# bacpop/Pansim

Hardware: AMD Instinct MI355X
Metric: generations/sec (higher is better)
Workload: dtype u8

## Files before the change

pansim_amd/csrc/acc_kernels.h:

```cpp
#pragma once

#include "ps_common.h"

struct acc_dims { uint32_t N, G, W, GW; };

__global__ void acc_init_kernel(uint64_t *accG, uint64_t *accI, const uint8_t *init_vec, acc_dims d)
{
    const uint64_t t = (uint64_t)blockIdx.x * blockDim.x + threadIdx.x;
    const uint64_t nG = (uint64_t)d.G * d.W, nI = (uint64_t)d.N * d.GW;
    if (t < nG) {
        const uint32_t g = (uint32_t)(t / d.W), w = (uint32_t)(t % d.W);
        const uint32_t nb = min(64u, d.N - w * 64u);
        const uint64_t m = (nb == 64u) ? ~0ull : ((1ull << nb) - 1ull);
        accG[t] = init_vec[g] ? m : 0ull;
    } else if (t < nG + nI) {
        const uint64_t u = t - nG;
        const uint32_t gw = (uint32_t)(u % d.GW);
        uint64_t word = 0;
        for (uint32_t b = 0; b < 64; b++) {
            const uint32_t g = gw * 64u + b;
            if (g < d.G && init_vec[g]) word |= 1ull << b;
        }
        accI[u] = word;
    }
// ... 66 lines not shown
    const uint32_t i = (uint32_t)(t / d.GW), gw = (uint32_t)(t % d.GW);
    const uint32_t p = DO_GATHER ? a.idx[i] : i;
    if (DO_GATHER && a.idx_out && gw == 0) a.idx_out[i] = p;
    uint64_t word = a.srcI[(uint64_t)p * d.GW + gw];
    if (DO_MUT && WT) {
        const uint4 *thr = (const uint4 *)(a.gene_thr + (size_t)gw * 64u);
        uint32_t lt[2] = { 0u, 0u };
#pragma unroll
        for (uint32_t j = 0; j < 16u; j++) {
            const ps_u4 r = ps_philox(gw * 16u + j, i, a.gen, PS_STREAM_ACC_MUT, a.k0, a.k1);
            const uint4 t = thr[j];
            const uint32_t b = 4u * j;
            lt[b >> 5] |= ((r.x < t.x ? 1u : 0u) | (r.y < t.y ? 2u : 0u) | (r.z < t.z ? 4u : 0u) | (r.w < t.w ? 8u : 0u)) << (b & 31u);
        }
        word ^= ((uint64_t)lt[1] << 32) | lt[0];
    } else if (DO_MUT) {
        const uint32_t t0 = a.plan.n_comp > 0 ? a.plan.flip_thr[0] : 0u, t1 = a.plan.n_comp > 1 ? a.plan.flip_thr[1] : 0u;
        const uint64_t m0 = a.plan.n_comp > 0 ? ps_word_range_mask(gw, a.plan.comp_begin[0], a.plan.comp_end[0]) : 0ull;
        const uint64_t m1 = a.plan.n_comp > 1 ? ps_word_range_mask(gw, a.plan.comp_begin[1], a.plan.comp_end[1]) : 0ull;
        uint32_t lt0[2] = { 0u, 0u }, lt1[2] = { 0u, 0u };
#pragma unroll
        for (uint32_t j = 0; j < 16u; j++) {
            const ps_u4 r = ps_philox(gw * 16u + j, i, a.gen, PS_STREAM_ACC_MUT, a.k0, a.k1);
            const uint32_t w[4] = { r.x, r.y, r.z, r.w };
#pragma unroll
            for (uint32_t k = 0; k < 4u; k++) {
                const uint32_t b = 4u * j + k;
                lt0[b >> 5] |= (w[k] < t0 ? 1u : 0u) << (b & 31u);
                lt1[b >> 5] |= (w[k] < t1 ? 1u : 0u) << (b & 31u);
            }
        }
        const uint64_t f0 = ((uint64_t)lt0[1] << 32) | lt0[0], f1 = ((uint64_t)lt1[1] << 32) | lt1[0];
        word ^= (f1 & m1) | (f0 & m0 & ~m1);
    }
    a.dstI[t] = word;
    if (a.snapI) a.snapI[t] = word;
}

struct acc_hgt_args {
    const uint64_t *srcI;
    uint64_t *dstI;
    acc_dims d;
    uint32_t n_comp;
    uint32_t gb[PS_MAX_COMP], ge[PS_MAX_COMP];
    const uint32_t *ptab[PS_MAX_COMP];
    uint32_t kmin[PS_MAX_COMP], plen[PS_MAX_COMP];
    uint32_t *work_ctr;
    uint32_t gen, k0, k1;
    uint32_t *bins, *counts;
    uint32_t bin_cap;
    uint32_t parts, rows_per_part;
    uint32_t part_magic;
    uint32_t *scratch;
    unsigned long long *ovf_img;
    uint32_t *overflow_flag;
    uint16_t *list_scratch;
    uint32_t list_stride;
    uint32_t dn_lo, dn_cnt;
    uint32_t bin_prio;
    const uint16_t *wq[PS_MAX_COMP];
    const uint64_t *wnz[PS_MAX_COMP];
    uint32_t pref_off;
};

__device__ __forceinline__ uint32_t ps_hgt_count(const acc_hgt_args &a, uint32_t c, uint32_t dn)
{
    if (!a.ptab[c]) return 0u;
    const ps_u4 r = ps_philox(dn, 0u, a.gen, PS_STREAM_HGT_COUNT | (c << 8), a.k0, a.k1);
    uint32_t lo = 0, hi = a.plen[c];
    while (lo < hi) {
        const uint32_t mid = (lo + hi) >> 1;
        if (a.ptab[c][mid] <= r.x) lo = mid + 1u; else hi = mid;
    }
    if (lo >= a.plen[c]) lo = a.plen[c] - 1u;
    return a.kmin[c] + lo;
}

__global__ void __launch_bounds__(256) acc_snapshot_kernel(const uint64_t *copy_src, uint64_t *copy_dst, uint64_t words)
{
    for (uint64_t w = (uint64_t)blockIdx.x * blockDim.x + threadIdx.x; w < words; w += (uint64_t)gridDim.x * blockDim.x)
        copy_dst[w] = copy_src[w];
}

__device__ __forceinline__ uint32_t ps_wave_gene_list(const uint64_t *row, uint32_t GW, uint32_t gb, uint32_t ge,
                                                      uint16_t *list, uint32_t lane)
{
    uint32_t base = 0;
    for (uint32_t gw0 = gb >> 6; gw0 * 64u < ge; gw0 += 64u) {
        const uint32_t gw = gw0 + lane;
        uint64_t word = 0;
        if (gw * 64u < ge && gw < GW) {
            word = row[gw];
            const uint32_t lo = gw * 64u;
            if (lo < gb) word &= ~0ull << (gb - lo);
            if (lo + 64u > ge) word &= (ge - lo >= 64u) ? ~0ull : ((1ull << (ge - lo)) - 1ull);
        }
        const uint32_t pc = __popcll(word);
        uint32_t incl = pc;
        for (int off = 1; off < 64; off <<= 1) {
            const uint32_t t = __shfl_up(incl, off, 64);
            if ((int)lane >= off) incl += t;
        }
        uint32_t pos = base + incl - pc;
        while (word) {
            const uint32_t b = (uint32_t)__builtin_ctzll(word);
            word &= word - 1ull;
            list[pos++] = (uint16_t)(gw * 64u + b);
        }
        base += __shfl(incl, 63, 64);
    }
    return base;
}

__device__ __forceinline__ uint32_t ps_wave_gene_list_w(const uint64_t *row, uint32_t GW, uint32_t G, const uint64_t *wnz, const uint16_t *wq,
                                                        uint16_t *list, uint32_t *pref, uint32_t lane, uint32_t *total)
{
    uint32_t base = 0, wbase = 0;
    for (uint32_t gw0 = 0; gw0 * 64u < G; gw0 += 64u) {
        const uint32_t gw = gw0 + lane;
        uint64_t word = 0;
        if (gw < GW) word = row[gw] & wnz[gw];
        const uint32_t pc = __popcll(word);
        uint32_t ws = 0;
        for (uint64_t t = word; t; t &= t - 1ull) ws += wq[gw * 64u + (uint32_t)__builtin_ctzll(t)];
        uint32_t incl = pc, wincl = ws;
        for (int off = 1; off < 64; off <<= 1) {
            const uint32_t t = __shfl_up(incl, off, 64), u = __shfl_up(wincl, off, 64);
            if ((int)lane >= off) { incl += t; wincl += u; }
        }
        uint32_t pos = base + incl - pc, run = wbase + wincl - ws;
        while (word) {
            const uint32_t g = gw * 64u + (uint32_t)__builtin_ctzll(word);
            word &= word - 1ull;
            run += wq[g];
            list[pos] = (uint16_t)g;
            pref[pos++] = run;
        }
        base += __shfl(incl, 63, 64);
        wbase += __shfl(wincl, 63, 64);
    }
    *total = wbase;
    return base;
}
__device__ __forceinline__ uint32_t ps_weighted_pick(const uint32_t *pref, uint32_t n, uint32_t total, uint32_t word)
{
    const uint32_t x = ps_mulhi(word, total);
    uint32_t lo = 0, hi = n - 1u;
    while (lo < hi) {
        const uint32_t mid = (lo + hi) >> 1;
        if (pref[mid] > x) hi = mid; else lo = mid + 1u;
    }
    return lo;
}

template <bool WT = false>
__global__ void __launch_bounds__(64) acc_hgt_donor_wave_kernel(acc_hgt_args a)
{
    extern __shared__ __attribute__((aligned(16))) uint16_t lds_list[];
    uint16_t *glist = a.list_scratch ? a.list_scratch + (uint64_t)blockIdx.x * a.list_stride : lds_list;
    uint32_t *pref = (uint32_t *)(glist + a.pref_off);
    uint32_t wtotal = 0;
    const acc_dims d = a.d;
    const uint32_t lane = threadIdx.x;
    const uint32_t items = a.n_comp * a.dn_cnt;
    for (;;) {
        uint32_t item = 0;
        if (lane == 0) item = atomicAdd(a.work_ctr, 1u);
        item = __builtin_amdgcn_readfirstlane(item);
        if (item >= items) break;
        const uint32_t c = item / a.dn_cnt, dn = a.dn_lo + item % a.dn_cnt;
        const uint32_t k = ps_hgt_count(a, c, dn);
        if (k == 0u) continue;
        __threadfence_block();
        const uint32_t n = WT ? ps_wave_gene_list_w(a.srcI + (uint64_t)dn * d.GW, d.GW, d.G, a.wnz[c], a.wq[c], glist, pref, lane, &wtotal)
                              : ps_wave_gene_list(a.srcI + (uint64_t)dn * d.GW, d.GW, a.gb[c], a.ge[c], glist, lane);
        __threadfence_block();
        if (n == 0u) continue;
        const uint32_t stream = PS_STREAM_HGT | (c << 8);
        for (uint32_t jp = lane; 2u * jp < k; jp += 64u) {
            const ps_u4 r = ps_philox(jp, dn, a.gen, stream, a.k0, a.k1);
#pragma unroll
            for (uint32_t h = 0; h < 2u; h++) {
                if (2u * jp + h >= k) break;
                uint32_t rc = ps_mulhi(h ? r.z : r.x, d.N - 1u);
                rc += (rc >= dn) ? 1u : 0u;
                const uint32_t gene = glist[WT ? ps_weighted_pick(pref, n, wtotal, h ? r.w : r.y) : ps_mulhi(h ? r.w : r.y, n)];
                atomicOr((unsigned long long *)&a.dstI[(uint64_t)rc * d.GW + (gene >> 6)], 1ull << (gene & 63u));
            }
        }
    }
}

#ifndef PS_HGT_BIN_BLOCKS
#define PS_HGT_BIN_BLOCKS 2u
#endif
template <bool WT = false>
__global__ void __launch_bounds__(256) acc_hgt_donor_bin_kernel(acc_hgt_args a)
{
    extern __shared__ __attribute__((aligned(16))) uint32_t sc_lds[];
    uint32_t *fill = sc_lds;
    uint16_t *glist = a.list_scratch ? a.list_scratch + (uint64_t)blockIdx.x * a.list_stride
                                     : (uint16_t *)(sc_lds + ((a.parts + 3u) & ~3u));
    __shared__ uint32_t sh_n;
    __shared__ uint32_t sh_total;
    const uint32_t *pref = (const uint32_t *)(glist + a.pref_off);
    const acc_dims d = a.d;
    const uint32_t tid = threadIdx.x, lane = tid & 63u;
    const uint32_t items = a.n_comp * a.dn_cnt;
    const uint32_t cap = a.bin_cap;
    if (a.bin_prio >= 3u) __builtin_amdgcn_s_setprio(3);
    else if (a.bin_prio == 2u) __builtin_amdgcn_s_setprio(2);
    else if (a.bin_prio == 1u) __builtin_amdgcn_s_setprio(1);
    uint32_t *mybins = a.bins + (uint64_t)blockIdx.x * a.parts * cap;
    for (uint32_t q = tid; q < a.parts; q += blockDim.x) fill[q] = 0u;
    for (uint32_t item = blockIdx.x; item < items; item += gridDim.x) {
        __syncthreads();
        const uint32_t c = item / a.dn_cnt, dn = a.dn_lo + item % a.dn_cnt;
        const uint32_t k = ps_hgt_count(a, c, dn);
        if (k == 0u) continue;
        if (tid < 64u) {
            uint32_t tot = 0;
            const uint32_t m = WT ? ps_wave_gene_list_w(a.srcI + (uint64_t)dn * d.GW, d.GW, d.G, a.wnz[c], a.wq[c], glist, (uint32_t *)(glist + a.pref_off), lane, &tot)
                                  : ps_wave_gene_list(a.srcI + (uint64_t)dn * d.GW, d.GW, a.gb[c], a.ge[c], glist, lane);
            if (tid == 0) { sh_n = m; if (WT) sh_total = tot; }
            __threadfence_block();
        }
        __syncthreads();
        const uint32_t n = sh_n;
        if (n == 0u) continue;
        const uint32_t wtotal = WT ? sh_total : 0u;
        const uint32_t stream = PS_STREAM_HGT | (c << 8);
        auto place = [&](uint32_t rc, uint32_t gene, uint32_t part, uint32_t pos) {
            if (pos < cap) mybins[(uint64_t)part * cap + pos] = ((rc - part * a.rows_per_part) << 16) | gene;
            else atomicOr(&a.ovf_img[(uint64_t)rc * d.GW + (gene >> 6)], 1ull << (gene & 63u));
        };
        constexpr uint32_t NBK = PS_HGT_BIN_BLOCKS;
        for (uint32_t jp = tid; 2u * jp < k; jp += NBK * blockDim.x) {
            uint32_t wr[2u * NBK], wg[2u * NBK];
            bool ok[2u * NBK];
#pragma unroll
            for (uint32_t b = 0; b < NBK; b++) {
                const uint32_t jb = jp + b * blockDim.x;
                const ps_u4 r = ps_philox(jb, dn, a.gen, stream, a.k0, a.k1);
                wr[2u * b] = r.x; wg[2u * b] = r.y; wr[2u * b + 1u] = r.z; wg[2u * b + 1u] = r.w;
                ok[2u * b] = 2u * jb < k;
                ok[2u * b + 1u] = 2u * jb + 1u < k;
            }
            uint32_t rc[2u * NBK], gene[2u * NBK], part[2u * NBK], pos[2u * NBK];
#pragma unroll
            for (uint32_t e = 0; e < 2u * NBK; e++) {
                rc[e] = ps_mulhi(wr[e], d.N - 1u);
                rc[e] += (rc[e] >= dn) ? 1u : 0u;
                gene[e] = glist[WT ? ps_weighted_pick(pref, n, wtotal, wg[e]) : ps_mulhi(wg[e], n)];
                part[e] = ps_mulhi(rc[e], a.part_magic);
            }
#pragma unroll
            for (uint32_t e = 0; e < 2u * NBK; e++) pos[e] = ok[e] ? atomicAdd(&fill[part[e]], 1u) : 0u;
#pragma unroll
            for (uint32_t e = 0; e < 2u * NBK; e++)
                if (ok[e]) place(rc[e], gene[e], part[e], pos[e]);
        }
    }
    __syncthreads();
    for (uint32_t q = tid; q < a.parts; q += blockDim.x) {
        a.counts[(uint64_t)blockIdx.x * a.parts + q] = min(fill[q], cap);
    }
}

__global__ void __launch_bounds__(1024) acc_hgt_apply_kernel(acc_hgt_args a, uint32_t donor_blocks, uint32_t n_slices)
{
    extern __shared__ uint32_t lrow[];
    const acc_dims d = a.d;
// ... 913 lines not shown
```

pansim_amd/csrc/core_kernels.h:

```cpp
#pragma once

#include "ps_common.h"

#include <type_traits>

#define PS_SWEEP_MAX_GENS 2
struct core_sweep_args {
    uint8_t *state;
    uint8_t *out;
    const uint32_t *idx;
    const uint32_t *idx_next[PS_SWEEP_MAX_GENS - 1];
    const uint32_t *idxT;
    uint32_t N, pitch, cpr, rows;
    uint32_t site_offset;
    uint32_t gen, k0, k1;
    ps_core_plan plan;
    uint32_t *overflow_flag;
    unsigned long long *stamps;
    uint32_t *work_ctr;
    uint32_t launch_parity;
    uint32_t nt;
    uint32_t qcap;
    uint32_t qcap_limit;
    uint32_t *wide_flags;
// ... 200 lines not shown
                                                     uint32_t k, uint32_t nE, uint32_t vm)
{
    const uint32_t c1 = __builtin_amdgcn_bitop3_b32(p1, p2, p3, 0x01) & vm;
    uint32_t lt;
    switch (nE) {
    case 1: lt = __builtin_amdgcn_bitop3_b32(p0, p5, p4, 0x01); break;
    case 2: lt = __builtin_amdgcn_bitop3_b32(p0, p5, p4, 0x03); break;
    case 3: lt = __builtin_amdgcn_bitop3_b32(p0, p5, p4, 0x07); break;
    case 4: lt = __builtin_amdgcn_bitop3_b32(p0, p5, p4, 0x0F); break;
    case 5: lt = __builtin_amdgcn_bitop3_b32(p0, p5, p4, 0x1F); break;
    case 6: lt = __builtin_amdgcn_bitop3_b32(p0, p5, p4, 0x3F); break;
    case 7: lt = __builtin_amdgcn_bitop3_b32(p0, p5, p4, 0x7F); break;
    default: lt = 0xFFFFFFFFu; break;
    }
    ps_class_words o;
    o.dec = k ? c1 & __builtin_amdgcn_bitop3_b32(p0, p5, p4, 0x07) : 0u;
    o.res = c1 & lt & ~o.dec;
    return o;
}

struct ps_apply_words { uint32_t y0, y1, ya, yb, yc; };
PS_HD uint32_t ps_bfi(uint32_t m, uint32_t a, uint32_t b)
{
#if defined(__HIP_DEVICE_COMPILE__) && __has_builtin(__builtin_amdgcn_bitop3_b32)
    return __builtin_amdgcn_bitop3_b32(m, a, b, 0xCA);
#else
    return (a & m) | (b & ~m);
#endif
}
__device__ __forceinline__ ps_apply_words ps_apply_prepare(uint32_t dec, uint32_t p4, uint32_t p5)
{
    const uint32_t r1 = p5 >> 1, r2 = p4 >> 2, l1 = p5 << 1, l2 = dec << 2;
    ps_apply_words o;
    o.y0 = ps_bfi(0x01010101u, p4, ps_bfi(0x02020202u, l1, l2));
    o.y1 = ps_bfi(0x02020202u, p4, ps_bfi(0x04040404u, l1, l2));
    o.ya = ps_bfi(0x09090909u, r2, ps_bfi(0x12121212u, r1, dec));
    o.yb = ps_bfi(0x12121212u, r2, ps_bfi(0x24242424u, r1, dec));
    o.yc = ps_bfi(0x24242424u, r2, ps_bfi(0x48484848u, r1, dec));
    return o;
}
template <uint32_t SLOT>
__device__ __forceinline__ uint32_t ps_apply_dword(const ps_apply_words &y, uint32_t d)
{
    constexpr uint32_t sh = SLOT == 0u ? 0u : SLOT == 1u ? 1u : SLOT == 2u ? 0u : SLOT == 3u ? 1u : SLOT == 4u ? 2u : SLOT == 5u ? 3u : SLOT == 6u ? 4u : 5u;
    const uint32_t src = SLOT == 0u ? y.y0 : SLOT == 1u ? y.y1 : (SLOT == 2u || SLOT == 5u) ? y.ya : (SLOT == 3u || SLOT == 6u) ? y.yb : y.yc;
    const uint32_t f = (src >> sh) & 0x07070707u;
    const uint32_t allele = __builtin_amdgcn_perm(0x00080402u, 0u, f);
    const uint32_t mask = __builtin_amdgcn_perm(0x00FFFFFFu, 0u, f);
    return ps_bfi(mask, allele, d);
}
template <uint32_t H>
__device__ __forceinline__ void ps_apply_row(const ps_apply_words &y, uint4 &d)
{
    d.x = ps_apply_dword<4u * H + 0u>(y, d.x);
    d.y = ps_apply_dword<4u * H + 1u>(y, d.y);
    d.z = ps_apply_dword<4u * H + 2u>(y, d.z);
    d.w = ps_apply_dword<4u * H + 3u>(y, d.w);
}

__device__ __forceinline__ uint32_t ps_push_scan(uint32_t w0, uint32_t w1, uint16_t *q, uint32_t lane, uint32_t qcap)
{
    const uint32_t c0 = (uint32_t)__popc(w0), c = c0 + (uint32_t)__popc(w1);
    const uint32_t incl = ps_wave_scan_incl(c);
    const uint32_t qn = __builtin_amdgcn_readlane(incl, 63);
    if (qn <= qcap) {
        uint16_t *qp = q + (incl - c) - 1, *qp1 = qp + c0;
        const uint32_t tag = lane << 6;
        for (uint32_t m = w0; m; m &= m - 1u) *++qp = (uint16_t)(tag | (uint32_t)__builtin_ctz(m));
        for (uint32_t m = w1; m; m &= m - 1u) *++qp1 = (uint16_t)(tag | 32u | (uint32_t)__builtin_ctz(m));
    }
    return qn;
}
__device__ __forceinline__ uint32_t ps_entry_cell(uint32_t ent)
{
    const uint32_t cell = ((ent & 3u) << 2) | ((ent >> 3) & 3u), row = ((ent >> 2) & 1u) | ((ent >> 4) & 2u);
    return (row << 10) | ((ent >> 2) & 0x3F0u) | cell;
}

PS_HD uint32_t ps_gather_dword(uint32_t lane, uint32_t m) { return lane + 64u * m; }
PS_HD uint32_t ps_gather_child(uint32_t lane, uint32_t m, uint32_t b) { return 4u * ps_gather_dword(lane, m) + b; }
PS_HD uint32_t ps_gather_source(uint32_t child, uint32_t parent, uint32_t N, uint32_t pitch)
{
    return child < N ? parent : (N < pitch - 1u ? N : pitch - 1u);
}

__device__ __forceinline__ uint32_t ps_pack4(uint32_t b0, uint32_t b1, uint32_t b2, uint32_t b3)
{
    return __builtin_amdgcn_perm(b1, b0, 0x0c0c0400u) | __builtin_amdgcn_perm(b3, b2, 0x04000c0cu);
}

#ifdef PS_STAMP
#define PS_T(k) do { unsigned long long t_; asm volatile("s_waitcnt lgkmcnt(0)\n\ts_memtime %0\n\ts_waitcnt lgkmcnt(0)" : "=s"(t_) :: "memory"); st_acc[k] += t_ - st_last; st_last = t_; } while (0)
#else
#define PS_T(k) do { } while (0)
#endif
#ifndef PS_WAVE_LB
#define PS_WAVE_LB 6
#endif
#ifndef PS_WAVE_PREFETCH
#define PS_WAVE_PREFETCH 0
#endif
__host__ __device__ constexpr uint32_t ps_queue_bytes(uint32_t qcap) { return (qcap * 2u + 15u) & ~15u; }
__host__ __device__ constexpr uint32_t ps_wave_lds(uint32_t qcap) { return PS_BATCH_ROWS * 1024u + ps_queue_bytes(qcap); }

template <bool DO_GATHER, bool DO_MUT, bool DO_HR, bool NT = false, bool WT = false, uint32_t T = 1>
__global__ void __launch_bounds__(256, T > 1 ? 4 : PS_WAVE_LB) core_sweep_wave_kernel(core_sweep_args a)
{
    static_assert(T >= 1 && T <= PS_SWEEP_MAX_GENS, "generations per pass");
    static_assert(T == 1 || (DO_GATHER && (DO_MUT || DO_HR)), "several generations per pass: the gather + events form only");
#ifdef PS_STAMP
    unsigned long long st_acc[8] = { 0, 0, 0, 0, 0, 0, 0, 0 };
    unsigned long long st_last;
    asm volatile("s_memtime %0\n\ts_waitcnt lgkmcnt(0)" : "=s"(st_last) :: "memory");
#endif
#ifdef PS_GROUP_TIMES
    const unsigned long long gt_start = __builtin_amdgcn_s_memrealtime();
#endif
    constexpr uint32_t PS_ROWS = PS_BATCH_ROWS;
    extern __shared__ __attribute__((aligned(16))) uint8_t lds[];
    const uint32_t wave = threadIdx.x >> 6, lane = threadIdx.x & 63u;
    uint8_t *rowbuf = lds + wave * ps_wave_lds(a.qcap);
    uint16_t *q = (uint16_t *)(rowbuf + PS_ROWS * 1024u);
    const ps_core_plan pl = a.plan;
    const uint32_t nE = 3u * pl.k + pl.R;
    constexpr bool events = DO_MUT || DO_HR;
    const bool has_chunk = lane < a.cpr;
    const uint32_t i0 = lane * 16u;
    const uint32_t ld_off = has_chunk ? i0 : 0u;
    const uint32_t nvalid = (i0 >= a.N) ? 0u : min(16u, a.N - i0);
    const uint32_t vm = ps_valid_word(nvalid);

    uint32_t pidx[T][16];
    if (DO_GATHER) {
#pragma unroll
        for (uint32_t t = 0; t < T; t++) {
            const uint32_t *ix = t ? a.idx_next[t ? t - 1u : 0u] : a.idx;
            const bool wide = ((uintptr_t)ix & 15u) == 0u;
#pragma unroll
            for (uint32_t m = 0; m < 4; m++) {
                const uint32_t c0 = ps_gather_child(lane, m, 0u);
                if (wide && c0 + 4u <= a.N) {
                    const uint4 p4 = *(const uint4 *)(ix + c0);
                    pidx[t][4u * m] = p4.x, pidx[t][4u * m + 1u] = p4.y, pidx[t][4u * m + 2u] = p4.z, pidx[t][4u * m + 3u] = p4.w;
                } else {
#pragma unroll
                    for (uint32_t b = 0; b < 4; b++) pidx[t][4u * m + b] = ps_gather_source(c0 + b, c0 + b < a.N ? ix[c0 + b] : 0u, a.N, a.pitch);
                }
            }
        }
    }

    constexpr uint32_t PS_CHUNK = 3u;
    const uint32_t grp = blockIdx.x & 7u;
    const uint32_t off = a.site_offset & 3u, g0 = a.site_offset >> 2;
    const uint32_t batches = (a.rows + off + PS_ROWS - 1u) / PS_ROWS;
    const uint32_t b_lo = (uint32_t)((uint64_t)batches * grp / 8u), b_hi = (uint32_t)((uint64_t)batches * (grp + 1u) / 8u);
    uint32_t *ctr = a.work_ctr + (a.launch_parity * 8u + grp) * 32u;
    if (blockIdx.x < 8u && threadIdx.x == 0) a.work_ctr[((a.launch_parity ^ 1u) * 8u + blockIdx.x) * 32u] = 0u;
    uint32_t next_chunk = 0;
    if (lane == 0) next_chunk = __hip_atomic_fetch_add(ctr, 1u, __ATOMIC_RELAXED, __HIP_MEMORY_SCOPE_AGENT);
#if PS_WAVE_PREFETCH
    uint4 vn[PS_ROWS];
    uint32_t pf_batch = 0xFFFFFFFFu;
#pragma unroll
    for (uint32_t rr = 0; rr < PS_ROWS; rr++) vn[rr] = make_uint4(0, 0, 0, 0);
#endif
    for (;;) {
        const uint32_t chunk = __builtin_amdgcn_readfirstlane(next_chunk);
        if (b_lo + chunk * PS_CHUNK >= b_hi) break;
        if (lane == 0) next_chunk = __hip_atomic_fetch_add(ctr, 1u, __ATOMIC_RELAXED, __HIP_MEMORY_SCOPE_AGENT);
    for (uint32_t cb = 0; cb < PS_CHUNK; cb++) {
        const uint32_t batch = b_lo + chunk * PS_CHUNK + cb;
        if (batch >= b_hi) break;
        const int lr0 = (int)(batch * PS_ROWS) - (int)off;
        const uint32_t sg = g0 + batch;
        auto lrow = [&](uint32_t rr) -> uint32_t { return (uint32_t)min(max(lr0 + (int)rr, 0), (int)a.rows - 1); };
        uint4 v[PS_ROWS];
#if PS_WAVE_PREFETCH
        if (pf_batch == batch) {
#pragma unroll
            for (uint32_t rr = 0; rr < PS_ROWS; rr++) v[rr] = vn[rr];
        } else
#endif
#pragma unroll
        for (uint32_t rr = 0; rr < PS_ROWS; rr++)
            v[rr] = ps_load_row16(a.state + (size_t)lrow(rr) * a.pitch + ld_off, NT);
        if (DO_GATHER) {
#pragma unroll
            for (uint32_t rr = 0; rr < PS_ROWS; rr++) *(uint4 *)(rowbuf + rr * 1024u + i0) = v[rr];
            ps_wave_sync();
        }
        PS_T(0);

#pragma unroll
        for (uint32_t t = 0; t < T; t++) {
        const uint32_t gen = a.gen + t;
        uint32_t wl[2] = { 0u, 0u };
        ps_apply_words y[2] = {};
        if (events) {
            const ps_u4 A0 = ps_philox_l1a(2u * sg, lane, gen, a.k0, a.k1);
            const ps_u4 A1 = ps_philox_l1a(2u * sg + 1u, lane, gen, a.k0, a.k1);
            const ps_u4 B = ps_philox_l1b(sg, lane, gen, a.k0, a.k1);
            const ps_class_words c0 = ps_classes(A0.x, A0.y, A0.z, A0.w, B.x, B.z, pl.k, nE, vm);
            const ps_class_words c1 = ps_classes(A1.x, A1.y, A1.z, A1.w, B.y, B.w, pl.k, nE, vm);
            wl[0] = c0.res;
            wl[1] = c1.res;
            if (DO_MUT) {
                y[0] = ps_apply_prepare(c0.dec, B.x & c0.dec, B.z & c0.dec);
                y[1] = ps_apply_prepare(c1.dec, B.y & c1.dec, B.w & c1.dec);
            }
        }
        PS_T(2);
        constexpr bool ahead = T > 1 && DO_GATHER;
        uint32_t g[16] = {};
        auto gather = [&](uint32_t rr) {
#pragma unroll
            for (int k = 0; k < 16; k++) g[k] = rowbuf[rr * 1024u + pidx[t][k]];
        };
        if (ahead) gather(0u);
#pragma unroll
        for (uint32_t rr = 0; rr < PS_ROWS; rr++) {
            uint8_t *row = rowbuf + rr * 1024u;
            uint4 d = v[rr];
            if (DO_GATHER) {
                if (!ahead) gather(rr);
                uint32_t w[4];
#pragma unroll
                for (int m = 0; m < 4; m++) w[m] = ps_pack4(g[4 * m], g[4 * m + 1], g[4 * m + 2], g[4 * m + 3]);
                ps_wave_sync();
#pragma unroll
                for (uint32_t m = 0; m < 4; m++) *(uint32_t *)(row + 4u * ps_gather_dword(lane, m)) = w[m];
                if (events && DO_MUT) {
                    ps_wave_sync();
                    d = *(const uint4 *)(row + i0);
                }
                if (ahead && rr + 1u < PS_ROWS) {
                    __builtin_amdgcn_sched_barrier(0);
                    gather(rr + 1u);
                    __builtin_amdgcn_sched_barrier(0);
                }
            }
            if (events && DO_MUT) {
                if (rr & 1u) ps_apply_row<1u>(y[rr >> 1], d);
                else ps_apply_row<0u>(y[rr >> 1], d);
            }
            if (events && (DO_MUT || !DO_GATHER)) *(uint4 *)(row + i0) = d;
            __builtin_amdgcn_sched_barrier(0);
        }
        PS_T(1);
        const uint32_t qcap = a.qcap_limit ? min(a.qcap, a.qcap_limit) : a.qcap;
        uint32_t qn = 0;
        if (events) qn = ps_push_scan(wl[0], wl[1], q, lane, qcap);
        PS_T(3);
        ps_wave_sync();
#if PS_WAVE_PREFETCH
        if (t + 1u == T) {
            uint32_t nb = batch + 1u;
            if (cb + 1u >= PS_CHUNK || nb >= b_hi) nb = b_lo + (uint32_t)__builtin_amdgcn_readfirstlane(next_chunk) * PS_CHUNK;
            pf_batch = nb < b_hi ? nb : 0xFFFFFFFFu;
            if (nb < b_hi) {
                const int nlr0 = (int)(nb * PS_ROWS) - (int)off;
#pragma unroll
                for (uint32_t rr = 0; rr < PS_ROWS; rr++)
                    vn[rr] = ps_load_row16(a.state + (size_t)(uint32_t)min(max(nlr0 + (int)rr, 0), (int)a.rows - 1) * a.pitch + ld_off, NT);
            }
        }
#endif
        const bool redo = events && (qn > qcap || (DO_HR && 2u * qn > qcap));
        if (redo) {
#pragma unroll 1
            for (uint32_t rr = 0; rr < PS_ROWS; rr++) {
                uint8_t *row = rowbuf + rr * 1024u;
                const uint32_t site = 4u * sg + rr;
                const ps_u4 Ar = ps_philox_l1a(site >> 1, lane, gen, a.k0, a.k1);
                const ps_u4 Br = ps_philox_l1b(sg, lane, gen, a.k0, a.k1);
                uint32_t cmr = ps_cand_word(Ar, site, pl.cshift) & vm;
                uint32_t hm = 0;
                while (cmr) {
                    const uint32_t k = ps_bit_cell(__builtin_ctz(cmr)), cellidx = i0 + k;
                    cmr &= cmr - 1u;
                    uint32_t l2y = 0;
                    const ps_cell cell = ps_cell_events<WT>(a, Ar, Br, site, cellidx, gen, a.k0, a.k1, pl, l2y);
                    if (DO_MUT && cell.mut) row[cellidx] = (uint8_t)cell.mut;
                    if (DO_HR && cell.hr) hm |= 1u << k;
                }
                if (DO_HR) {
                    ps_wave_sync();
                    uint32_t dv[4] = { 0u, 0u, 0u, 0u };
                    for (uint32_t tmp = hm; tmp;) {
                        const uint32_t k = __builtin_ctz(tmp), cellidx = i0 + k;
                        tmp &= tmp - 1u;
                        const ps_u4 l2 = ps_philox(site, cellidx, gen, PS_STREAM_CORE_L2, a.k0, a.k1);
                        uint32_t donor = ps_mulhi(l2.y, a.N - 1u);
                        donor += (donor >= cellidx) ? 1u : 0u;
                        ps_set_byte(dv, k, (uint32_t)row[donor]);
                    }
                    ps_wave_sync();
                    for (uint32_t tmp = hm; tmp;) {
                        const uint32_t k = __builtin_ctz(tmp);
                        tmp &= tmp - 1u;
                        row[i0 + k] = (uint8_t)((dv[k >> 2] >> (8u * (k & 3u))) & 0xFFu);
                    }
                }
            }
            ps_wave_sync();
        } else if (events) {
            uint16_t *qh = q + qcap - 1u;
            for (uint32_t base = 0; base < qn; base += 64u) {
                const uint32_t e = base + lane;
                if (e < qn) {
                    const uint32_t ent = ps_entry_cell(q[e]);
                    const uint32_t cellidx = ent & 1023u, rr = ent >> 10;
                    const ps_u4 l2 = ps_philox(4u * sg + rr, cellidx, gen, PS_STREAM_CORE_L2, a.k0, a.k1);
                    const ps_cell cell = ps_classify_site<WT>(l2.x, pl, a, 4u * sg + rr);
                    if (DO_MUT && cell.mut) rowbuf[ent] = (uint8_t)cell.mut;
                    if (DO_HR) {
                        uint32_t out = 0;
                        if (cell.hr) {
                            uint32_t donor = ps_mulhi(l2.y, a.N - 1u);
                            donor += (donor >= cellidx) ? 1u : 0u;
                            out = donor | 0x8000u;
                        }
                        *(qh - e) = (uint16_t)out;
                    }
                }
            }
            if (DO_HR) {
                ps_wave_sync();
                for (uint32_t base = 0; base < qn; base += 64u) {
                    const uint32_t e = base + lane;
                    if (e < qn) {
                        const uint32_t h = *(qh - e);
                        if (h >> 15) *(qh - e) = (uint16_t)((uint32_t)rowbuf[(ps_entry_cell(q[e]) & 3072u) | (h & 1023u)] | 0x8000u);
                    }
                }
                ps_wave_sync();
                for (uint32_t base = 0; base < qn; base += 64u) {
                    const uint32_t e = base + lane;
                    if (e < qn) {
                        const uint32_t h = *(qh - e);
                        if (h >> 15) rowbuf[ps_entry_cell(q[e])] = (uint8_t)(h & 0xFFu);
                    }
                }
            }
            ps_wave_sync();
        }
        }
        PS_T(5);

        if (has_chunk) {
#pragma unroll
            for (uint32_t rr = 0; rr < PS_ROWS; rr++) {
                const int lr = lr0 + (int)rr;
                if (lr >= 0 && lr < (int)a.rows) {
                    const uint4 o = (DO_GATHER || events) ? *(const uint4 *)(rowbuf + rr * 1024u + i0) : v[rr];
                    ps_store_row16(a.out + (size_t)lr * a.pitch + i0, o, NT);
                }
            }
        }
        ps_wave_sync();
        PS_T(6);
    }
    }
#ifdef PS_STAMP
    if (lane == 0)
        for (int k = 0; k < 8; k++) atomicAdd((unsigned long long *)a.stamps + k, st_acc[k]);
#endif
#ifdef PS_GROUP_TIMES
    if (lane == 0) {
        atomicMax((unsigned long long *)a.stamps + 8 + grp, (unsigned long long)__builtin_amdgcn_s_memrealtime());
        atomicMax((unsigned long long *)a.stamps + 16 + grp, gt_start);
        if (blockIdx.x < 8 && wave == 0) ((unsigned long long *)a.stamps)[24 + grp] = gt_start;
    }
#endif
}

#ifndef PS_WCAP
#define PS_WCAP 1216u
#endif
#ifndef PS_WBPC
#define PS_WBPC 6
#endif
#ifndef PS_WLB
#define PS_WLB 6
#endif
#ifndef PS_WINDOW_NT_LOADS
#define PS_WINDOW_NT_LOADS 0
#endif
#define PS_WSTRIDE (PS_WCAP + 16u)
#define PS_WHR 64u
__host__ __device__ constexpr uint32_t ps_window_lds(uint32_t qcap) { return PS_BATCH_ROWS * PS_WSTRIDE + ps_queue_bytes(qcap) + PS_WHR * 6u; }

template <bool WT>
__device__ __forceinline__ uint32_t ps_donor_value(const core_sweep_args &a, const ps_core_plan &pl, const uint8_t *old_row,
                                                   uint32_t site, uint32_t donor, bool do_mut)
{
    uint32_t val = old_row[a.idx[donor]];
    if (do_mut) {
        const ps_u4 A = ps_philox_l1a(site >> 1, donor >> 4, a.gen, a.k0, a.k1);
        const uint32_t n = ps_cell_nibble(A, site, donor);
        if ((n >> pl.cshift) == 0u) {
            const ps_u4 B = ps_philox_l1b(site >> 2, donor >> 4, a.gen, a.k0, a.k1);
            const uint32_t code = ps_sym_code(4u * n + ps_cell_pair(B, site, donor), pl);
            if (code > 1u) {
                val = code;
            } else if (code == 1u) {
                const ps_u4 l2 = ps_philox(site, donor, a.gen, PS_STREAM_CORE_L2, a.k0, a.k1);
                const ps_cell cell = ps_classify_site<WT>(l2.x, pl, a, site);
                if (cell.mut) val = cell.mut;
            }
        }
    }
    return val;
}


template <bool DO_MUT, bool DO_HR, bool NT, bool WIDE, bool WT = false>
__global__ void __launch_bounds__(256, PS_WLB) core_sweep_window_kernel(core_sweep_args a)
{
    constexpr uint32_t PS_ROWS = PS_BATCH_ROWS;
    extern __shared__ __attribute__((aligned(16))) uint8_t lds[];
    const uint32_t wave = threadIdx.x >> 6, lane = threadIdx.x & 63u;
    uint8_t *rowbuf = lds + wave * ps_window_lds(a.qcap);
    uint16_t *q = (uint16_t *)(rowbuf + PS_ROWS * PS_WSTRIDE);
    uint32_t *hr_d = (uint32_t *)(rowbuf + PS_ROWS * PS_WSTRIDE + ps_queue_bytes(a.qcap));
    uint16_t *hr_e = (uint16_t *)(hr_d + PS_WHR);
    if (lane < PS_ROWS) *(uint4 *)(rowbuf + lane * PS_WSTRIDE + PS_WCAP) = make_uint4(0, 0, 0, 0);
    const ps_core_plan pl = a.plan;
    const uint32_t segs = (a.N + 1023u) >> 10;
    const uint32_t grp = blockIdx.x & 7u;
    const uint32_t wg = __builtin_amdgcn_readfirstlane((blockIdx.x >> 3) * 4u + wave);
    const uint32_t sgm = wg % segs;
    if (wg < segs && lane == 0) a.work_ctr[(((a.launch_parity ^ 1u) * 8u + grp) * segs + wg) * 32u] = 0u;
    if (WIDE) {
        if (__builtin_amdgcn_readfirstlane(a.wide_flags[(a.gen & 1u) * 32u]) == 0u) return;
    } else if (blockIdx.x == 0 && threadIdx.x == 0) {
        a.wide_flags[((a.gen + 1u) & 1u) * 32u] = 0u;
    }
// ... 1592 lines not shown
```

pansim_amd/csrc/pansim_capi.hip:

```cpp
#include "../../include/pansim_hip.h"

#include <hip/hip_runtime.h>

#include <algorithm>
#include <charconv>
#include <chrono>
#include <condition_variable>
#include <mutex>
#include <cmath>
#include <cstdarg>
#include <cstdio>
#include <cstdlib>
#include <cstring>
#include <string>
#include <thread>
#include <type_traits>
#include <vector>

#include "acc_kernels.h"
#include "core_kernels.h"
#include "ps_common.h"

static thread_local std::string g_err;

// ... 1256 lines not shown
        const uint32_t n_slices = std::max(1u, p->hgt_slices ? p->hgt_slices : auto_slices);
        const uint64_t words = (uint64_t)p->d.N * p->d.GW;
        const uint64_t img_bytes = (uint64_t)n_slices * words * 8;
        double per_block = 0.0;
        for (int c = 0; c < p->aplan.n_comp; c++)
            if (a.ptab[c]) per_block += p->aplan.lam_rec[c] * (double)((a.dn_cnt + donor_blocks - 1) / donor_blocks);
        const double mean = per_block * (double)rows_per_part / (double)(p->d.N - 1);
        uint32_t cap = (uint32_t)(((uint64_t)(mean + 10.0 * std::sqrt(mean) + 64.0) + 63) & ~63ull);
        if (p->hgt_bin_cap) cap = std::min(cap, std::max(1u, p->hgt_bin_cap));
        const uint64_t bin_words = (uint64_t)donor_blocks * parts * cap;
        const uint64_t cnt_bytes = ((uint64_t)donor_blocks * parts * 4 + 255) & ~255ull;
        const uint64_t list_bytes = p->hgt_bin_list_in_global ? (((uint64_t)donor_blocks * list_u16 * sizeof(uint16_t) + 255) & ~255ull) : 0;
        const uint64_t need = img_bytes + bin_words * 4 + cnt_bytes + list_bytes;
        PSCHK(dev_grow(p->hgt_scratch, p->hgt_scratch_cap, need));
        if (!p->hgt_ovf_img) {
            HIPCHK(hipMalloc(&p->hgt_ovf_img, words * 8));
            HIPCHK(hipMemsetAsync(p->hgt_ovf_img, 0, words * 8, st));
        }
        a.ovf_img = (unsigned long long *)p->hgt_ovf_img;
        a.scratch = (uint32_t *)p->hgt_scratch;
        a.bins = (uint32_t *)((uint8_t *)p->hgt_scratch + img_bytes);
        a.counts = (uint32_t *)((uint8_t *)p->hgt_scratch + img_bytes + bin_words * 4);
        a.parts = parts;
        a.rows_per_part = rows_per_part;
        a.part_magic = (uint32_t)(4294967296ull / rows_per_part) + 1u;
        a.bin_cap = cap;
        a.srcI = p->I[p->cur];
        a.dstI = p->I[p->cur];
        a.bin_prio = p->hgt_bin_prio;
        if (list_bytes) {
            a.list_scratch = (uint16_t *)((uint8_t *)p->hgt_scratch + img_bytes + bin_words * 4 + cnt_bytes);
            a.list_stride = list_u16;
        }
        const uint32_t dlds = ((parts + 3u) & ~3u) * 4u + (list_bytes ? 0u : list_lds);
        auto bin_kern = wt ? acc_hgt_donor_bin_kernel<true> : acc_hgt_donor_bin_kernel<false>;
        if (dlds > 64 * 1024)
            HIPCHK(hipFuncSetAttribute((const void *)bin_kern, hipFuncAttributeMaxDynamicSharedMemorySize, (int)dlds));
        hipLaunchKernelGGL(bin_kern, dim3(donor_blocks), dim3(256), dlds, st, a);
        const bool in_gap = st_gap && ev_bin && record_after_apply && !p->exchange_beside_sweep;
        hipStream_t run = st;
        if (in_gap) {
            HIPCHK(hipEventRecord(ev_bin, st));
            HIPCHK(hipStreamWaitEvent(st_gap, ev_bin, 0));
            run = st_gap;
        } else if (wait_before_apply) HIPCHK(hipStreamWaitEvent(st, wait_before_apply, 0));
        auto kern = acc_hgt_apply_kernel;
        if (lds > 64 * 1024)
            HIPCHK(hipFuncSetAttribute((const void *)kern, hipFuncAttributeMaxDynamicSharedMemorySize, (int)lds));
        hipLaunchKernelGGL(kern, dim3(parts * n_slices), dim3(p->hgt_apply_threads), lds, run, a, donor_blocks, n_slices);
        if (record_after_apply && (!sharded || p->exchange_beside_sweep)) {
            HIPCHK(hipEventRecord(record_after_apply, run));
            if (in_gap) HIPCHK(hipStreamWaitEvent(st, record_after_apply, 0));
            record_after_apply = nullptr;
            run = st;
        }
        st = run;
        if (!sharded && p->fuse_counts_out) {
            acc_hgt_reduce_rows_kernel<<<(uint32_t)((p->d.N + 3) / 4), 256, 0, st>>>((const uint64_t *)p->hgt_scratch, p->I[p->cur], p->d,
                                                                                    n_slices, (unsigned long long *)p->hgt_ovf_img,
                                                                                    p->fuse_counts_out, p->fuse_logw_out);
            counts_left = true;
        } else
        acc_hgt_reduce_kernel<<<(uint32_t)((words + 255) / 256), 256, 0, st>>>((const uint64_t *)p->hgt_scratch,
                                                                              sharded ? p->d_delta : p->I[p->cur], words, n_slices,
                                                                              sharded ? 1 : 0, (unsigned long long *)p->hgt_ovf_img);
    } else {
        a.srcI = have_snapshot ? p->I_snap : p->I[1 - p->cur];
        a.dstI = sharded ? p->d_delta : p->I[p->cur];
        if (sharded) HIPCHK(hipMemsetAsync(p->d_delta, 0, mat_words * 8, st));
        uint32_t grid = std::min(items, 256u * 32u);
        if (p->hgt_events_per_thread) {
            const double expected_here = expected * (double)a.dn_cnt / (double)p->d.N;
            const uint64_t want = (uint64_t)(expected_here / ((double)p->hgt_events_per_thread * 64.0)) + 1;
            grid = (uint32_t)std::min<uint64_t>(std::max<uint64_t>(want, 1), grid);
        }
        uint32_t dyn_lds = list_lds;
        if (p->hgt_list_in_global) {
            const uint64_t need = (uint64_t)grid * list_u16 * sizeof(uint16_t);
            PSCHK(dev_grow(p->hgt_scratch, p->hgt_scratch_cap, need));
            a.list_scratch = (uint16_t *)p->hgt_scratch;
            a.list_stride = list_u16;
            dyn_lds = 0;
        }
        auto wave_kern = wt ? acc_hgt_donor_wave_kernel<true> : acc_hgt_donor_wave_kernel<false>;
        if (dyn_lds > 64 * 1024)
            HIPCHK(hipFuncSetAttribute((const void *)wave_kern, hipFuncAttributeMaxDynamicSharedMemorySize, (int)dyn_lds));
        hipLaunchKernelGGL(wave_kern, dim3(grid), dim3(64), dyn_lds, st, a);
    }
    HIPCHK(hipGetLastError());
    if (sharded) {
        if (p->exchange) {
            const std::string prev = g_err;
            g_err.clear();
            const int rc = p->exchange(p->exchange_ctx, p->d_delta, p->delta_words, (void *)st);
            if (rc != 0) {
                const std::string inner = g_err;
                return ps_fail(PS_ERR_STATE, "the HGT delta exchange failed (%d)%s%s", rc, inner.empty() ? "" : ": ", inner.c_str());
            }
            g_err = prev;
        }
        if (p->fuse_counts_out) {
            acc_or_rows_kernel<<<(uint32_t)((p->d.N + 3) / 4), 256, 0, st>>>(p->I[p->cur], p->d_delta, p->d, p->fuse_counts_out, p->fuse_logw_out);
            counts_left = true;
        } else
        acc_or_kernel<<<(uint32_t)((mat_words + 255) / 256), 256, 0, st>>>(p->I[p->cur], p->d_delta, mat_words);
        HIPCHK(hipGetLastError());
    }
    if (record_after_apply) {
        HIPCHK(hipEventRecord(record_after_apply, st));
        if (st != p->stream_of_call) HIPCHK(hipStreamWaitEvent(p->stream_of_call, record_after_apply, 0));
    }
    p->g_valid = false;
    p->counts_fresh = counts_left;
    p->edit_epoch++;
    return PS_OK;
}

extern "C" int ps_set_donor_shard(ps_population *p, uint32_t shard_rank, uint32_t shard_count, ps_exchange_fn fn, void *ctx)
{
    if (!p) return ps_fail(PS_ERR_INVALID, "null handle");
    if (p->cfg.core) return ps_fail(PS_ERR_INVALID, "donor shards apply to the accessory matrix (HGT, population.rs:544-751)");
    if (shard_count < 1 || shard_rank >= shard_count) return ps_fail(PS_ERR_INVALID, "bad donor shard %u of %u", shard_rank, shard_count);
    const uint64_t N = p->cfg.pop_size;
    if (shard_count == 1) {
        p->donor_lo = 0;
        p->donor_cnt = 0;
        p->exchange = nullptr;
        p->exchange_ctx = nullptr;
        return PS_OK;
    }
    const uint64_t lo = N * shard_rank / shard_count, hi = N * ((uint64_t)shard_rank + 1) / shard_count;
    if (hi <= lo) return ps_fail(PS_ERR_INVALID, "more donor shards than individuals");
    p->donor_lo = (uint32_t)lo;
    p->donor_cnt = (uint32_t)(hi - lo);
    p->exchange = fn;
    p->exchange_ctx = ctx;
    return PS_OK;
}

static int upload_idx(ps_population *p, const uint32_t *sample)
{
    const uint64_t N = p->cfg.pop_size;
    for (uint64_t i = 0; i < N; i++)
        if (sample[i] >= N) return ps_fail(PS_ERR_INVALID, "parent index %u out of range", sample[i]);
    HIPCHK(hipMemcpyAsync(p->d_idx, sample, N * sizeof(uint32_t), hipMemcpyHostToDevice, p->stream));
    return PS_OK;
}

static int step_device(ps_population *p, const uint32_t *d_idx, uint32_t gen, bool ga, bool mu, bool hr,
                       hipStream_t st, uint32_t *idx_out = nullptr, bool parents_sorted = false)
{
    if (p->cfg.core) return launch_core_sweep(p, d_idx, gen, ga, mu, hr, st, parents_sorted);
    if (ga || mu) PSCHK(launch_acc_step(p, d_idx, gen, ga, mu, st, idx_out));
    if (hr) PSCHK(launch_acc_hgt(p, gen, st));
    return PS_OK;
}

extern "C" int ps_next_generation(ps_population *p, const uint32_t *sample)
{
    if (!p || !sample) return ps_fail(PS_ERR_INVALID, "null argument");
    PSCHK(use_device(p));
    PSCHK(upload_idx(p, sample));
    PSCHK(step_device(p, p->d_idx, 0, true, false, false, p->stream));
    p->rows_overridden = true;
    return sync_checked(p);
}

// ... 2863 lines not shown
```

Baseline: 3287.

## Swizzle LDS row layout in core sweep and specialize HGT wave kernel for LDS lists

The core sweep kernel now keeps each row buffer in LDS in a permuted dword order that matches the gather lane mapping. Gathered bytes are packed straight into registers and stored once per chunk, which removes an intermediate store, a wave sync and a reload. Every byte index into the row buffer (mutations, recombination donors, queue fixups, output reload) goes through a physical-index mapping, and parent indices are pre-translated. Separately, the HGT donor wave kernel gets a compile-time LDS variant that uses address-space-3 pointers and LDS-only fences instead of full block fences, and its two-event inner loop is unrolled branch-free. The main risk is index-mapping bugs and extra ALU work per access.

New measurement: 2983. -9.3%, worse.

```diff
diff --git a/pansim_amd/csrc/acc_kernels.h b/pansim_amd/csrc/acc_kernels.h
--- a/pansim_amd/csrc/acc_kernels.h
+++ b/pansim_amd/csrc/acc_kernels.h
@@ -172,8 +172,9 @@
         copy_dst[w] = copy_src[w];
 }
 
+template <class L16>
 __device__ __forceinline__ uint32_t ps_wave_gene_list(const uint64_t *row, uint32_t GW, uint32_t gb, uint32_t ge,
-                                                      uint16_t *list, uint32_t lane)
+                                                      L16 list, uint32_t lane)
 {
     uint32_t base = 0;
     for (uint32_t gw0 = gb >> 6; gw0 * 64u < ge; gw0 += 64u) {
@@ -202,8 +203,9 @@
     return base;
 }
 
+template <class L16, class L32>
 __device__ __forceinline__ uint32_t ps_wave_gene_list_w(const uint64_t *row, uint32_t GW, uint32_t G, const uint64_t *wnz, const uint16_t *wq,
-                                                        uint16_t *list, uint32_t *pref, uint32_t lane, uint32_t *total)
+                                                        L16 list, L32 pref, uint32_t lane, uint32_t *total)
 {
     uint32_t base = 0, wbase = 0;
     for (uint32_t gw0 = 0; gw0 * 64u < G; gw0 += 64u) {
@@ -232,7 +234,8 @@
     *total = wbase;
     return base;
 }
-__device__ __forceinline__ uint32_t ps_weighted_pick(const uint32_t *pref, uint32_t n, uint32_t total, uint32_t word)
+template <class L32>
+__device__ __forceinline__ uint32_t ps_weighted_pick(L32 pref, uint32_t n, uint32_t total, uint32_t word)
 {
     const uint32_t x = ps_mulhi(word, total);
     uint32_t lo = 0, hi = n - 1u;
@@ -243,12 +246,10 @@
     return lo;
 }
 
-template <bool WT = false>
-__global__ void __launch_bounds__(64) acc_hgt_donor_wave_kernel(acc_hgt_args a)
-{
-    extern __shared__ __attribute__((aligned(16))) uint16_t lds_list[];
-    uint16_t *glist = a.list_scratch ? a.list_scratch + (uint64_t)blockIdx.x * a.list_stride : lds_list;
-    uint32_t *pref = (uint32_t *)(glist + a.pref_off);
+#define PS_LDS_AS __attribute__((address_space(3)))
+template <bool WT, bool LDS_LIST, class L16, class L32>
+__device__ __forceinline__ void ps_hgt_wave_items(const acc_hgt_args &a, L16 glist, L32 pref)
+{
     uint32_t wtotal = 0;
     const acc_dims d = a.d;
     const uint32_t lane = threadIdx.x;
@@ -261,23 +262,37 @@
         const uint32_t c = item / a.dn_cnt, dn = a.dn_lo + item % a.dn_cnt;
         const uint32_t k = ps_hgt_count(a, c, dn);
         if (k == 0u) continue;
-        __threadfence_block();
+        if (LDS_LIST) __builtin_amdgcn_fence(__ATOMIC_SEQ_CST, "workgroup", "local"); else __threadfence_block();
         const uint32_t n = WT ? ps_wave_gene_list_w(a.srcI + (uint64_t)dn * d.GW, d.GW, d.G, a.wnz[c], a.wq[c], glist, pref, lane, &wtotal)
                               : ps_wave_gene_list(a.srcI + (uint64_t)dn * d.GW, d.GW, a.gb[c], a.ge[c], glist, lane);
-        __threadfence_block();
+        if (LDS_LIST) __builtin_amdgcn_fence(__ATOMIC_SEQ_CST, "workgroup", "local"); else __threadfence_block();
         if (n == 0u) continue;
         const uint32_t stream = PS_STREAM_HGT | (c << 8);
         for (uint32_t jp = lane; 2u * jp < k; jp += 64u) {
             const ps_u4 r = ps_philox(jp, dn, a.gen, stream, a.k0, a.k1);
-#pragma unroll
-            for (uint32_t h = 0; h < 2u; h++) {
-                if (2u * jp + h >= k) break;
-                uint32_t rc = ps_mulhi(h ? r.z : r.x, d.N - 1u);
-                rc += (rc >= dn) ? 1u : 0u;
-                const uint32_t gene = glist[WT ? ps_weighted_pick(pref, n, wtotal, h ? r.w : r.y) : ps_mulhi(h ? r.w : r.y, n)];
-                atomicOr((unsigned long long *)&a.dstI[(uint64_t)rc * d.GW + (gene >> 6)], 1ull << (gene & 63u));
-            }
-        }
+            const bool two = 2u * jp + 1u < k;
+            uint32_t rc0 = ps_mulhi(r.x, d.N - 1u), rc1 = ps_mulhi(r.z, d.N - 1u);
+            rc0 += (rc0 >= dn) ? 1u : 0u;
+            rc1 += (rc1 >= dn) ? 1u : 0u;
+            const uint32_t i0 = WT ? ps_weighted_pick(pref, n, wtotal, r.y) : ps_mulhi(r.y, n);
+            const uint32_t i1 = WT ? ps_weighted_pick(pref, n, wtotal, r.w) : ps_mulhi(r.w, n);
+            const uint32_t gene0 = glist[i0], gene1 = glist[two ? i1 : i0];
+            rc1 = two ? rc1 : rc0;
+            atomicOr((unsigned long long *)&a.dstI[(uint64_t)rc0 * d.GW + (gene0 >> 6)], 1ull << (gene0 & 63u));
+            atomicOr((unsigned long long *)&a.dstI[(uint64_t)rc1 * d.GW + (gene1 >> 6)], 1ull << (gene1 & 63u));
+        }
+    }
+}
+template <bool WT = false, bool LDS_LIST = true>
+__global__ void __launch_bounds__(64) acc_hgt_donor_wave_kernel(acc_hgt_args a)
+{
+    if (LDS_LIST) {
+        extern __shared__ __attribute__((aligned(16))) uint16_t lds_list[];
+        PS_LDS_AS uint16_t *glist = (PS_LDS_AS uint16_t *)lds_list;
+        ps_hgt_wave_items<WT, true>(a, glist, (PS_LDS_AS uint32_t *)(glist + a.pref_off));
+    } else {
+        uint16_t *glist = a.list_scratch + (uint64_t)blockIdx.x * a.list_stride;
+        ps_hgt_wave_items<WT, false>(a, glist, (uint32_t *)(glist + a.pref_off));
     }
 }
 
diff --git a/pansim_amd/csrc/core_kernels.h b/pansim_amd/csrc/core_kernels.h
--- a/pansim_amd/csrc/core_kernels.h
+++ b/pansim_amd/csrc/core_kernels.h
@@ -306,6 +306,21 @@
 PS_HD uint32_t ps_gather_source(uint32_t child, uint32_t parent, uint32_t N, uint32_t pitch)
 {
     return child < N ? parent : (N < pitch - 1u ? N : pitch - 1u);
+}
+
+PS_HD uint32_t ps_row_phys_dword(uint32_t d) { return ((d & 3u) << 6) | ((d >> 2) & 63u); }
+PS_HD uint32_t ps_row_phys_byte(uint32_t cell) { return (ps_row_phys_dword(cell >> 2) << 2) | (cell & 3u); }
+PS_HD uint32_t ps_row_logical_dword(uint32_t pd) { return ((pd & 63u) << 2) | ((pd >> 6) & 3u); }
+PS_HD uint32_t ps_row_logical_byte(uint32_t pb) { return (ps_row_logical_dword(pb >> 2) << 2) | (pb & 3u); }
+__device__ __forceinline__ void ps_row_store_chunk(uint8_t *row, uint32_t lane, const uint4 &d)
+{
+    uint32_t *r = (uint32_t *)row;
+    r[ps_gather_dword(lane, 0u)] = d.x, r[ps_gather_dword(lane, 1u)] = d.y, r[ps_gather_dword(lane, 2u)] = d.z, r[ps_gather_dword(lane, 3u)] = d.w;
+}
+__device__ __forceinline__ uint4 ps_row_load_chunk(const uint8_t *row, uint32_t lane)
+{
+    const uint32_t *r = (const uint32_t *)row;
+    return make_uint4(r[ps_gather_dword(lane, 0u)], r[ps_gather_dword(lane, 1u)], r[ps_gather_dword(lane, 2u)], r[ps_gather_dword(lane, 3u)]);
 }
 
 __device__ __forceinline__ uint32_t ps_pack4(uint32_t b0, uint32_t b1, uint32_t b2, uint32_t b3)
@@ -362,7 +377,7 @@
             const bool wide = ((uintptr_t)ix & 15u) == 0u;
 #pragma unroll
             for (uint32_t m = 0; m < 4; m++) {
-                const uint32_t c0 = ps_gather_child(lane, m, 0u);
+                const uint32_t c0 = i0 + 4u * m;
                 if (wide && c0 + 4u <= a.N) {
                     const uint4 p4 = *(const uint4 *)(ix + c0);
                     pidx[t][4u * m] = p4.x, pidx[t][4u * m + 1u] = p4.y, pidx[t][4u * m + 2u] = p4.z, pidx[t][4u * m + 3u] = p4.w;
@@ -371,6 +386,8 @@
                     for (uint32_t b = 0; b < 4; b++) pidx[t][4u * m + b] = ps_gather_source(c0 + b, c0 + b < a.N ? ix[c0 + b] : 0u, a.N, a.pitch);
                 }
             }
+#pragma unroll
+            for (uint32_t k = 0; k < 16; k++) pidx[t][k] = ps_row_phys_byte(pidx[t][k]);
         }
     }
 
@@ -411,7 +428,7 @@
             v[rr] = ps_load_row16(a.state + (size_t)lrow(rr) * a.pitch + ld_off, NT);
         if (DO_GATHER) {
 #pragma unroll
-            for (uint32_t rr = 0; rr < PS_ROWS; rr++) *(uint4 *)(rowbuf + rr * 1024u + i0) = v[rr];
+            for (uint32_t rr = 0; rr < PS_ROWS; rr++) ps_row_store_chunk(rowbuf + rr * 1024u, lane, v[rr]);
             ps_wave_sync();
         }
         PS_T(0);
@@ -448,27 +465,18 @@
             uint4 d = v[rr];
             if (DO_GATHER) {
                 if (!ahead) gather(rr);
-                uint32_t w[4];
-#pragma unroll
-                for (int m = 0; m < 4; m++) w[m] = ps_pack4(g[4 * m], g[4 * m + 1], g[4 * m + 2], g[4 * m + 3]);
-                ps_wave_sync();
-#pragma unroll
-                for (uint32_t m = 0; m < 4; m++) *(uint32_t *)(row + 4u * ps_gather_dword(lane, m)) = w[m];
-                if (events && DO_MUT) {
-                    ps_wave_sync();
-                    d = *(const uint4 *)(row + i0);
-                }
-                if (ahead && rr + 1u < PS_ROWS) {
-                    __builtin_amdgcn_sched_barrier(0);
-                    gather(rr + 1u);
-                    __builtin_amdgcn_sched_barrier(0);
-                }
+                d.x = ps_pack4(g[0], g[1], g[2], g[3]);
+                d.y = ps_pack4(g[4], g[5], g[6], g[7]);
+                d.z = ps_pack4(g[8], g[9], g[10], g[11]);
+                d.w = ps_pack4(g[12], g[13], g[14], g[15]);
+                if (ahead && rr + 1u < PS_ROWS) gather(rr + 1u);
             }
             if (events && DO_MUT) {
                 if (rr & 1u) ps_apply_row<1u>(y[rr >> 1], d);
                 else ps_apply_row<0u>(y[rr >> 1], d);
             }
-            if (events && (DO_MUT || !DO_GATHER)) *(uint4 *)(row + i0) = d;
+            if (DO_GATHER) ps_wave_sync();
+            if (DO_GATHER || events) ps_row_store_chunk(row, lane, d);
             __builtin_amdgcn_sched_barrier(0);
         }
         PS_T(1);
@@ -505,7 +513,7 @@
                     cmr &= cmr - 1u;
                     uint32_t l2y = 0;
                     const ps_cell cell = ps_cell_events<WT>(a, Ar, Br, site, cellidx, gen, a.k0, a.k1, pl, l2y);
-                    if (DO_MUT && cell.mut) row[cellidx] = (uint8_t)cell.mut;
+                    if (DO_MUT && cell.mut) row[ps_row_phys_byte(cellidx)] = (uint8_t)cell.mut;
                     if (DO_HR && cell.hr) hm |= 1u << k;
                 }
                 if (DO_HR) {
@@ -517,13 +525,13 @@
                         const ps_u4 l2 = ps_philox(site, cellidx, gen, PS_STREAM_CORE_L2, a.k0, a.k1);
                         uint32_t donor = ps_mulhi(l2.y, a.N - 1u);
                         donor += (donor >= cellidx) ? 1u : 0u;
-                        ps_set_byte(dv, k, (uint32_t)row[donor]);
+                        ps_set_byte(dv, k, (uint32_t)row[ps_row_phys_byte(donor)]);
                     }
                     ps_wave_sync();
                     for (uint32_t tmp = hm; tmp;) {
                         const uint32_t k = __builtin_ctz(tmp);
                         tmp &= tmp - 1u;
-                        row[i0 + k] = (uint8_t)((dv[k >> 2] >> (8u * (k & 3u))) & 0xFFu);
+                        row[ps_row_phys_byte(i0 + k)] = (uint8_t)((dv[k >> 2] >> (8u * (k & 3u))) & 0xFFu);
                     }
                 }
             }
@@ -537,7 +545,7 @@
                     const uint32_t cellidx = ent & 1023u, rr = ent >> 10;
                     const ps_u4 l2 = ps_philox(4u * sg + rr, cellidx, gen, PS_STREAM_CORE_L2, a.k0, a.k1);
                     const ps_cell cell = ps_classify_site<WT>(l2.x, pl, a, 4u * sg + rr);
-                    if (DO_MUT && cell.mut) rowbuf[ent] = (uint8_t)cell.mut;
+                    if (DO_MUT && cell.mut) rowbuf[(ent & 3072u) | ps_row_phys_byte(cellidx)] = (uint8_t)cell.mut;
                     if (DO_HR) {
                         uint32_t out = 0;
                         if (cell.hr) {
@@ -555,7 +563,7 @@
                     const uint32_t e = base + lane;
                     if (e < qn) {
                         const uint32_t h = *(qh - e);
-                        if (h >> 15) *(qh - e) = (uint16_t)((uint32_t)rowbuf[(ps_entry_cell(q[e]) & 3072u) | (h & 1023u)] | 0x8000u);
+                        if (h >> 15) *(qh - e) = (uint16_t)((uint32_t)rowbuf[(ps_entry_cell(q[e]) & 3072u) | ps_row_phys_byte(h & 1023u)] | 0x8000u);
                     }
                 }
                 ps_wave_sync();
@@ -563,7 +571,10 @@
                     const uint32_t e = base + lane;
                     if (e < qn) {
                         const uint32_t h = *(qh - e);
-                        if (h >> 15) rowbuf[ps_entry_cell(q[e])] = (uint8_t)(h & 0xFFu);
+                        if (h >> 15) {
+                            const uint32_t ent = ps_entry_cell(q[e]);
+                            rowbuf[(ent & 3072u) | ps_row_phys_byte(ent & 1023u)] = (uint8_t)(h & 0xFFu);
+                        }
                     }
                 }
             }
@@ -577,7 +588,7 @@
             for (uint32_t rr = 0; rr < PS_ROWS; rr++) {
                 const int lr = lr0 + (int)rr;
                 if (lr >= 0 && lr < (int)a.rows) {
-                    const uint4 o = (DO_GATHER || events) ? *(const uint4 *)(rowbuf + rr * 1024u + i0) : v[rr];
+                    const uint4 o = (DO_GATHER || events) ? ps_row_load_chunk(rowbuf + rr * 1024u, lane) : v[rr];
                     ps_store_row16(a.out + (size_t)lr * a.pitch + i0, o, NT);
                 }
             }
diff --git a/pansim_amd/csrc/pansim_capi.hip b/pansim_amd/csrc/pansim_capi.hip
--- a/pansim_amd/csrc/pansim_capi.hip
+++ b/pansim_amd/csrc/pansim_capi.hip
@@ -1362,7 +1362,8 @@
             a.list_stride = list_u16;
             dyn_lds = 0;
         }
-        auto wave_kern = wt ? acc_hgt_donor_wave_kernel<true> : acc_hgt_donor_wave_kernel<false>;
+        auto wave_kern = a.list_scratch ? (wt ? acc_hgt_donor_wave_kernel<true, false> : acc_hgt_donor_wave_kernel<false, false>)
+                                        : (wt ? acc_hgt_donor_wave_kernel<true, true> : acc_hgt_donor_wave_kernel<false, true>);
         if (dyn_lds > 64 * 1024)
             HIPCHK(hipFuncSetAttribute((const void *)wave_kern, hipFuncAttributeMaxDynamicSharedMemorySize, (int)dyn_lds));
         hipLaunchKernelGGL(wave_kern, dim3(grid), dim3(64), dyn_lds, st, a);
```
